# IvanPopov/video-flow-ml

Hardware: AMD Instinct MI355X
Metric: flow-fields/sec @1080p seq5 MOF_sintel (higher is better)
Workload: dtype mixed (per-layer MFMA count, f32 accumulate): {"corr": 1, "update_block.encoder.convf1": 1, "update_block.encoder.convf2": 1, "update_block.gru.convq1.iter": "2a", "update_block.gru.convzr1.iter": 1, "update_block.gru.convzr2.iter": 1, "update_block.mask.0": 1, "update_block.mask.2": 1, "update_bloc

## Files before the change

### include/vfml.h

```cpp
#ifndef VFML_H
#define VFML_H
#include <stddef.h>
#include <stdint.h>

#ifdef __cplusplus
extern "C" {
#endif

#define VFML_ABI_VERSION 25

enum {
  VFML_EPI_NONE = 0,
  VFML_EPI_RELU = 1,
  VFML_EPI_TANH = 2,
  VFML_EPI_SIGMOID = 3,
  VFML_EPI_TANH_RELU = 4,
  VFML_EPI_GRU_ZR = 5,
  VFML_EPI_GRU_Q = 6,
  VFML_EPI_ADD_AUX = 7,
};

enum { VFML_FMT_F32 = 0, VFML_FMT_S16 = 1,
       VFML_FMT_F16 = 2 };

// ... 58 lines not shown
                        const float* res_stats, int n, int hw, int c, float* out, int out_fmt, void* stream);

int vfml_avgpool2x2(const float* x, int n, int h, int w, int c, float* out, void* stream);

int vfml_corr_lookup(const float* const* pyr, const int32_t* hl, const int32_t* wl,
                     const int32_t* ld, int levels, int radius, int nmaps, int q_per_map,
                     const float* coords, int ld_coords, float* out, int ld_out, int out_fmt, int vol_fmt, int vol_tile,
                     void* stream);
#define VFML_VOL_F16_LEVELS(m) (0x100 | (m))

int vfml_corr_lookup_indirect(const float* const* table, const int32_t* hl, const int32_t* wl, const int32_t* ld,
                              int levels, int radius, int nmaps, int q_per_map, const float* coords, int ld_coords,
                              float* out, int ld_out, int out_fmt, int vol_fmt, int vol_tile, void* stream);
int vfml_corr_lookup_indirect_bidir(const float* const* table, const int32_t* hl, const int32_t* wl, const int32_t* ld,
                                    int levels, int radius, int nmaps, int q_per_map, const float* coords, int ld_coords,
                                    int dir_coords, float* out, int ld_out, int dir_out, int dir_tab, int out_fmt, int vol_fmt,
                                    int vol_tile, void* stream);
int vfml_ptr_table_set(void* table, const void* const* ptrs, int n, void* stream);

int vfml_flow_rows7(const float* flow, int n, int h, int w, float* rows, void* stream);

int vfml_conv3x3_c64(const float* in, int ld_in, int n, int h, int w, const void* w_hi, const void* w_lo, int kp, float w_scale,
                     const float* bias, float* out, int ldo, double* stats_part, void* stream);

int vfml_flow_half(const float* flow, int n, int h, int w, const void* w1_hi, int kp1, float w1_scale, const float* b1,
                   const void* w2_hi, int kp2, float w2_scale, const float* b2, float* out, int ld_out, void* stream);

int vfml_tapsum3x3(const float* t, int ld_t, const float* bias, int n, int h, int w, float* out, int parts, int64_t part_stride,
                   void* stream);
int vfml_tapsum3x3_update(const float* t, int ld_t, const float* bias, int n, int h, int w, int parts, int64_t part_stride,
                          float* coords1, float* flow_a, int ld_a, float* flow_b, int ld_b, int fmt_b, void* stream);

int vfml_coords_update(float* coords1, const float* delta, int n, int h, int w,
                       float* flow_a, int ld_a, float* flow_b, int ld_b, int fmt_b, void* stream);
int vfml_coords_init(float* coords1, int n, int h, int w, void* stream);

int vfml_convex_upsample(const float* coords1, int ch, const float* mask, int ld_mask,
                         int h, int w, float* out, void* stream);

int64_t vfml_instnorm_finalize_workspace_bytes(int chunks, int c);
int vfml_instnorm_finalize(const double* part, int n, int chunks, int c, int hw, float eps, float* stats,
                           void* workspace, int64_t workspace_bytes, void* stream);

int vfml_stem7x7s2_chunks(int h, int w);
int vfml_stem7x7s2(const float* frames, int n, int h, int w, const void* w_hi, const void* w_lo, float w_scale,
                   const float* bias, float* out, double* stats_part, void* stream);
// ... 39 lines not shown
```

### video-flow-ml_amd/vfml/csrc/enc_conv.hip

```cpp
#include "conv_split_common.h"

namespace {

constexpr int EC_C = 64;
constexpr int EC_TH = 4, EC_TW = 32;
constexpr int EC_PR = EC_TH + 2, EC_PW = EC_TW + 2;
constexpr int EC_PIX = 272;
constexpr int EC_PATCH = EC_PR * EC_PW * EC_PIX;
constexpr int EC_VLD = EC_C + 4;
constexpr int EC_LDS = EC_PATCH;
constexpr int EC_K = 9 * EC_C;
constexpr int EC_NS = EC_K / 32;
static_assert(EC_TH * EC_TW * EC_VLD * 4 <= EC_PATCH, "the result tile fits where the patch was");

struct EncConvArgs {
  const char* in;
  const _Float16* whi; const _Float16* wlo;
  const float* bias;
  float* out; int ldo;
  double* stats_part;
  int ld_in, n, H, W, tiles_x, tiles_y;
  float w_inv;
};

__global__ __launch_bounds__(256, 2) void enc_conv3x3_c64_kernel(const EncConvArgs a) {
  extern __shared__ __attribute__((aligned(16))) char smem[];
  float* sV = reinterpret_cast<float*>(smem);

  const int t = threadIdx.x, lane = t & 63;
  const int wave = __builtin_amdgcn_readfirstlane(t >> 6);
  const int r4 = lane & 15, u4 = lane >> 4;
  const int tiles_img = a.tiles_x * a.tiles_y;
  const int total = a.n * tiles_img;

  h16x8 bh[EC_NS], bl[EC_NS];
  static_for<EC_NS>([&](auto sc) {
    constexpr int s = decltype(sc)::value;
    bh[s] = *reinterpret_cast<const h16x8*>(a.whi + (16 * wave + r4) * EC_K + s * 32 + u4 * 8);
    bl[s] = *reinterpret_cast<const h16x8*>(a.wlo + (16 * wave + r4) * EC_K + s * 32 + u4 * 8);
  });
  f32x4 bias4 = {0.f, 0.f, 0.f, 0.f};
  if (a.bias) bias4 = *reinterpret_cast<const f32x4*>(a.bias + 16 * wave + 4 * u4);

  for (int tile = blockIdx.x; tile < total; tile += gridDim.x) {
    const int img = tile / tiles_img, tl = tile - img * tiles_img;
    const int ty = tl / a.tiles_x, tx = tl - ty * a.tiles_x;
    const int oy0 = ty * EC_TH, ox0 = tx * EC_TW;

    constexpr int NPC = EC_PR * EC_PW * 16;
    constexpr int NPT = (NPC + 255) / 256;
    const __amdgpu_buffer_rsrc_t rin = __builtin_amdgcn_make_buffer_rsrc(
        const_cast<char*>(a.in) + (int64_t)img * a.H * a.W * a.ld_in * 4, 0, a.H * a.W * a.ld_in * 4, 0x00020000);
    u32x4 pv[NPT];
    static_for<NPT>([&](auto qc) {
      constexpr int q = decltype(qc)::value;
      const int c = min(t + 256 * q, NPC - 1);
      const int p = c >> 4, piece = c & 15;
      const int py = p / EC_PW, px = p - py * EC_PW;
      const int iy = oy0 - 1 + py, ix = ox0 - 1 + px;
      const bool ok = (unsigned)iy < (unsigned)a.H && (unsigned)ix < (unsigned)a.W;
      pv[q] = bload16(rin, ok ? ((iy * a.W + ix) * a.ld_in) * 4 + piece * 16 : (int)0x80000000);
    });
    __syncthreads();
    static_for<NPT>([&](auto qc) {
      constexpr int q = decltype(qc)::value;
      const int c = t + 256 * q;
      if (c < NPC) *reinterpret_cast<u32x4*>(smem + (c >> 4) * EC_PIX + (c & 15) * 16) = pv[q];
    });
    __syncthreads();

    f32x4 acc[8];
#pragma unroll
    for (int m = 0; m < 8; ++m) acc[m] = f32x4{0.f, 0.f, 0.f, 0.f};
    const char* al = smem + r4 * EC_PIX + u4 * 32;
    static_for<2>([&](auto hc) {
      constexpr int mh = decltype(hc)::value;
      static_for<EC_NS>([&](auto sc) {
        constexpr int s = decltype(sc)::value;
        constexpr int cb = s / 9, ky = (s % 9) / 3, kx = s % 3;
#pragma unroll
        for (int mm = 0; mm < 4; ++mm) {
          const int m = 4 * mh + mm;
          const char* p = al + (((m >> 1) + ky) * EC_PW + 16 * (m & 1) + kx) * EC_PIX + cb * 128;
          const h16x8 ah = *reinterpret_cast<const h16x8*>(p);
          const h16x8 alo = *reinterpret_cast<const h16x8*>(p + 16);
          acc[m] = __builtin_amdgcn_mfma_f32_16x16x32_f16(bh[s], ah, acc[m], 0, 0, 0);
          acc[m] = __builtin_amdgcn_mfma_f32_16x16x32_f16(bl[s], ah, acc[m], 0, 0, 0);
          acc[m] = __builtin_amdgcn_mfma_f32_16x16x32_f16(bh[s], alo, acc[m], 0, 0, 0);
        }
        if constexpr (s % 3 == 2) __builtin_amdgcn_sched_barrier(0);
// ... 17 lines not shown
      __syncthreads();
      const int row = t >> 6, ch = t & 63;
      const int oy = oy0 + row;
      if (oy < a.H) {
        double s1 = 0.0, s2 = 0.0;
        for (int x = 0; x < EC_TW; ++x) {
          float f = sV[(row * EC_TW + x) * EC_VLD + ch], g;
          asm("v_mov_b32 %0, %1" : "=v"(g) : "v"(f));
          const double v = (double)g;
          s1 += v;
          s2 += v * v;
        }
        const int64_t chunk = (((int64_t)img * a.H + oy) * a.W + ox0) >> 5;
        double* o = a.stats_part + (chunk * EC_C + ch) * 2;
        o[0] = s1;
        o[1] = s2;
      }
    }
  }
}

}

extern "C" int vfml_conv3x3_c64(const float* in, int ld_in, int n, int h, int w, const void* w_hi, const void* w_lo, int kp,
                                float w_scale, const float* bias, float* out, int ldo, double* stats_part, void* stream) {
  VFML_REQUIRE(in && w_hi && w_lo && out && n > 0 && h > 0 && w > 0, "vfml_conv3x3_c64: bad argument");
  VFML_REQUIRE(w % EC_TW == 0, "vfml_conv3x3_c64: the image width must be a multiple of %d (got %d)", EC_TW, w);
  VFML_REQUIRE(kp == EC_K && w_scale > 0.f, "vfml_conv3x3_c64: weight planes [64][%d] (VFML_KORDER_CBLOCK), got row pitch %d", EC_K, kp);
  VFML_REQUIRE((reinterpret_cast<uintptr_t>(in) & 31u) == 0 && ld_in >= EC_C && ld_in % 8 == 0 && vfml_aligned16(w_hi) &&
                   vfml_aligned16(w_lo) && vfml_aligned16(bias) && vfml_aligned16(out) && ldo >= EC_C && ldo % 4 == 0 &&
                   (reinterpret_cast<uintptr_t>(stats_part) & 7u) == 0,
               "vfml_conv3x3_c64: a 32-byte aligned split-row input (ld_in %% 8 == 0), 16-byte aligned weights / bias / output "
               "(ldo %% 4 == 0)");
  EncConvArgs a;
  a.in = reinterpret_cast<const char*>(in); a.ld_in = ld_in;
  a.whi = reinterpret_cast<const _Float16*>(w_hi); a.wlo = reinterpret_cast<const _Float16*>(w_lo);
  a.bias = bias; a.out = out; a.ldo = ldo; a.stats_part = stats_part;
  a.n = n; a.H = h; a.W = w; a.tiles_x = w / EC_TW; a.tiles_y = (h + EC_TH - 1) / EC_TH;
  a.w_inv = 1.0f / w_scale;
  const int64_t total = (int64_t)n * a.tiles_x * a.tiles_y;
  VFML_REQUIRE(total < (1ll << 31) && (int64_t)h * w * ld_in * 4 < (1ll << 31), "vfml_conv3x3_c64: an image of the input must stay below 2 GiB");
  const int grid = (int)(total < 512 ? total : 512);
  hipLaunchKernelGGL(enc_conv3x3_c64_kernel, dim3(grid), dim3(256), EC_LDS, reinterpret_cast<hipStream_t>(stream), a);
  return vfml_check_launch("vfml_conv3x3_c64");
}
```

### video-flow-ml_amd/vfml/csrc/norm_pool.hip

```cpp
#include <stdlib.h>
#include "vfml_common.h"

namespace {

__global__ void frames_u8_kernel(const uint8_t* __restrict__ src, int64_t npx, float scale, float shift,
                                 f32x4* __restrict__ dst) {
  for (int64_t p = (int64_t)blockIdx.x * blockDim.x + threadIdx.x; p < npx; p += (int64_t)gridDim.x * blockDim.x) {
    const uint8_t* s = src + p * 3;
    f32x4 v;
    v[0] = scale * ((float)s[0] / 255.0f) + shift;
    v[1] = scale * ((float)s[1] / 255.0f) + shift;
    v[2] = scale * ((float)s[2] / 255.0f) + shift;
    v[3] = 0.f;
    dst[p] = v;
  }
}

__global__ void frames_f32_kernel(const float* __restrict__ src, int n, int64_t hw, float scale, float shift,
                                  f32x4* __restrict__ dst) {
  const int64_t npx = (int64_t)n * hw;
  for (int64_t p = (int64_t)blockIdx.x * blockDim.x + threadIdx.x; p < npx; p += (int64_t)gridDim.x * blockDim.x) {
    const int64_t f = p / hw, q = p - f * hw;
    const float* s = src + f * 3 * hw + q;
    f32x4 v;
// ... 34 lines not shown
  extern __shared__ __attribute__((aligned(16))) char smem_raw[];
  double* sh = reinterpret_cast<double*>(smem_raw);
  if (pl < lanes) {
#pragma unroll
    for (int e = 0; e < 4; ++e) {
      sh[((int64_t)pl * c + g * 4 + e) * 2 + 0] = s[e];
      sh[((int64_t)pl * c + g * 4 + e) * 2 + 1] = q[e];
    }
  }
  __syncthreads();
  for (int ch = t; ch < c; ch += STAT_THREADS) {
    double ss = 0, qq = 0;
    for (int l = 0; l < lanes; ++l) {
      ss += vfml_lds_f64(&sh[((int64_t)l * c + ch) * 2 + 0]);
      qq += vfml_lds_f64(&sh[((int64_t)l * c + ch) * 2 + 1]);
    }
    double* o = part + (((int64_t)n * gridDim.x + chunk) * c + ch) * 2;
    o[0] = ss;
    o[1] = qq;
  }
}

constexpr int FINAL_THREADS = 256;
__global__ __launch_bounds__(FINAL_THREADS) void instnorm_final_kernel(const double* __restrict__ part, int n, int chunks,
                                                                      int c, int hw, float eps, float* __restrict__ stats) {
  __shared__ double sh[FINAL_THREADS][2];
  const int i = blockIdx.x;
  const int nn = i / c, ch = i - nn * c;
  const int t = threadIdx.x;
  const double* base = part + ((int64_t)nn * chunks * c + ch) * 2;
  double s = 0, q = 0;
  int k = t;
  for (; k + 3 * FINAL_THREADS < chunks; k += 4 * FINAL_THREADS) {
    const double* p0 = base + (int64_t)k * c * 2;
    const double* p1 = p0 + (int64_t)FINAL_THREADS * c * 2;
    const double* p2 = p1 + (int64_t)FINAL_THREADS * c * 2;
    const double* p3 = p2 + (int64_t)FINAL_THREADS * c * 2;
    const double a0 = p0[0], b0 = p0[1], a1 = p1[0], b1 = p1[1], a2 = p2[0], b2 = p2[1], a3 = p3[0], b3 = p3[1];
    s += a0; q += b0; s += a1; q += b1; s += a2; q += b2; s += a3; q += b3;
  }
  for (; k < chunks; k += FINAL_THREADS) {
    const double* p = base + (int64_t)k * c * 2;
    s += p[0];
    q += p[1];
  }
  sh[t][0] = s;
  sh[t][1] = q;
  __syncthreads();
  if (t == 0) {
    double ss = 0, qq = 0;
    for (int l = 0; l < FINAL_THREADS; ++l) {
      ss += vfml_lds_f64(&sh[l][0]);
      qq += vfml_lds_f64(&sh[l][1]);
    }
    const double mean = ss / hw;
    double var = qq / hw - mean * mean;
    if (var < 0) var = 0;
    stats[2 * i + 0] = (float)mean;
    stats[2 * i + 1] = (float)(1.0 / sqrt(var + (double)eps));
  }
}

constexpr int FOLD_SLICES = 64;
__global__ __launch_bounds__(256) void instnorm_fold_kernel(const double* __restrict__ part, int chunks, int c,
                                                            double* __restrict__ out) {
  __shared__ double sh[32][8][2];
  const int cgs = c / 8;
  const int sl = blockIdx.x % FOLD_SLICES, cg = (blockIdx.x / FOLD_SLICES) % cgs, nn = blockIdx.x / (FOLD_SLICES * cgs);
  const int ch = threadIdx.x & 7, lane = threadIdx.x >> 3;
  const int per = (chunks + FOLD_SLICES - 1) / FOLD_SLICES;
  const int k0 = sl * per, k1 = k0 + per < chunks ? k0 + per : chunks;
  const double* base = part + ((int64_t)nn * chunks * c + cg * 8 + ch) * 2;
  double s0 = 0, q0 = 0;
  for (int k = k0 + lane; k < k1; k += 32) {
    const double* p = base + (int64_t)k * c * 2;
    s0 += p[0];
    q0 += p[1];
  }
  sh[lane][ch][0] = s0;
  sh[lane][ch][1] = q0;
  __syncthreads();
  if (lane == 0) {
// ... 105 lines not shown
  return vfml_check_launch("vfml_frames_to_nhwc4");
}

extern "C" int64_t vfml_instnorm_workspace_bytes(int n, int hw, int c) {
  return (int64_t)n * stat_chunks(hw) * c * 2 * sizeof(double);
}

extern "C" int vfml_instnorm_stats(const float* x, int n, int hw, int c, float eps, float* stats, void* workspace,
                                   void* stream) {
  VFML_REQUIRE(x && stats && workspace, "vfml_instnorm_stats: null pointer");
  VFML_REQUIRE(n > 0 && hw > 0 && c > 0 && c % 4 == 0 && c <= 1024, "vfml_instnorm_stats: bad n/hw/c (c%%4==0, c<=1024)");
  VFML_REQUIRE(vfml_aligned16(x), "vfml_instnorm_stats: x must be 16-byte aligned");
  hipStream_t s = reinterpret_cast<hipStream_t>(stream);
  const int chunks = stat_chunks(hw);
  const int px = (hw + chunks - 1) / chunks;
  const int lanes = STAT_THREADS / (c / 4);
  VFML_REQUIRE(lanes >= 1, "vfml_instnorm_stats: too many channels");
  const size_t lds = (size_t)lanes * c * 2 * sizeof(double);
  VFML_REQUIRE(lds <= 64 * 1024, "vfml_instnorm_stats: LDS budget");
  hipLaunchKernelGGL(instnorm_partial_kernel, dim3(chunks, n), dim3(STAT_THREADS), lds, s, x, hw, c, px,
                     (double*)workspace);
  int rc = vfml_check_launch("vfml_instnorm_stats(partial)");
  if (rc) return rc;
  hipLaunchKernelGGL(instnorm_final_kernel, dim3(n * c), dim3(FINAL_THREADS), 0, s, (const double*)workspace, n, chunks, c, hw,
                     eps, stats);
  return vfml_check_launch("vfml_instnorm_stats(final)");
}

static bool finalize_folds(int chunks, int c) { return chunks >= 1024 && c % 8 == 0; }

extern "C" int64_t vfml_instnorm_finalize_workspace_bytes(int chunks, int c) {
  return finalize_folds(chunks, c) ? (int64_t)FOLD_SLICES * c * 16 : 0;
}

extern "C" int vfml_instnorm_finalize(const double* part, int n, int chunks, int c, int hw, float eps, float* stats,
                                      void* workspace, int64_t workspace_bytes, void* stream) {
  VFML_REQUIRE(part && stats && n > 0 && chunks > 0 && c > 0 && hw > 0, "vfml_instnorm_finalize: bad argument");
  hipStream_t st = reinterpret_cast<hipStream_t>(stream);
  if (finalize_folds(chunks, c)) {
    const int64_t per_frame = (int64_t)FOLD_SLICES * c * 16;
    VFML_REQUIRE(workspace && workspace_bytes >= per_frame && (reinterpret_cast<uintptr_t>(workspace) & 15u) == 0,
                 "vfml_instnorm_finalize: %d partials x %d channels fold through a workspace of >= %lld bytes (16-byte aligned); got %lld",
                 chunks, c, (long long)per_frame, (long long)(workspace ? workspace_bytes : 0));
    const int nmax = (int)(workspace_bytes / per_frame);
    for (int n0 = 0; n0 < n; n0 += nmax) {
      const int nb = n - n0 < nmax ? n - n0 : nmax;
      hipLaunchKernelGGL(instnorm_fold_kernel, dim3(nb * (c / 8) * FOLD_SLICES), dim3(256), 0, st,
                         part + (int64_t)n0 * chunks * c * 2, chunks, c, (double*)workspace);
      hipLaunchKernelGGL(instnorm_final_kernel, dim3(nb * c), dim3(FINAL_THREADS), 0, st, (const double*)workspace, nb,
                         FOLD_SLICES, c, hw, eps, stats + (int64_t)n0 * c * 2);
    }
    return vfml_check_launch("vfml_instnorm_finalize");
  }
  hipLaunchKernelGGL(instnorm_final_kernel, dim3(n * c), dim3(FINAL_THREADS), 0, st, part, n, chunks,
                     c, hw, eps, stats);
  return vfml_check_launch("vfml_instnorm_finalize");
}

extern "C" int vfml_instnorm_apply(const float* x, const float* stats, const float* res, const float* res_stats, int n,
                                   int hw, int c, float* out, int out_fmt, void* stream) {
  VFML_REQUIRE(x && stats && out, "vfml_instnorm_apply: null pointer");
  VFML_REQUIRE(n > 0 && hw > 0 && c > 0 && c % 4 == 0, "vfml_instnorm_apply: bad n/hw/c");
  VFML_REQUIRE(out_fmt == VFML_FMT_F32 || (out_fmt == VFML_FMT_S16 && c % 8 == 0 && (reinterpret_cast<uintptr_t>(out) & 31u) == 0 &&
                                            (!res || res_stats || (reinterpret_cast<uintptr_t>(res) & 31u) == 0)),
               "vfml_instnorm_apply: split-row output needs c %% 8 == 0 and 32-byte aligned out (and res)");
  VFML_REQUIRE(!(res_stats && !res), "vfml_instnorm_apply: res_stats without res");
  VFML_REQUIRE(vfml_aligned16(x) && vfml_aligned16(out) && vfml_aligned16(res), "vfml_instnorm_apply: alignment");
  hipStream_t s = reinterpret_cast<hipStream_t>(stream);
  const int64_t total4 = (int64_t)n * hw * (c / 4);
  const dim3 g(grid_for(total4, 256)), b(256);
  const bool s16 = out_fmt == VFML_FMT_S16;
#define VFML_APPLY(MODE, S16, R, RS)                                                                                      \
  hipLaunchKernelGGL((instnorm_apply_kernel<MODE, S16>), g, b, 0, s, (const f32x4*)x, stats, (const f32x4*)(R), RS, hw, c, \
                     total4, (f32x4*)out)
  if (!res) {
    if (s16) VFML_APPLY(0, true, nullptr, nullptr); else VFML_APPLY(0, false, nullptr, nullptr);
  } else if (!res_stats) {
// ... 19 lines not shown
```

### video-flow-ml_amd/vfml/hip.py

```python
import ctypes
import os
import subprocess
from ctypes import POINTER, c_char_p, c_double, c_float, c_int, c_int32, c_int64, c_void_p

import torch

_HERE = os.path.dirname(os.path.abspath(__file__))
LIB_PATH = os.environ.get("VFML_LIB") or os.path.join(_HERE, "libvfml_hip.so")
CSRC = os.path.join(_HERE, "csrc")
SOURCES = ["api.hip", "conv_gemm.hip", "conv_gemm_split.hip", "conv_gemm_tapx.hip", "stem.hip", "flow_half.hip", "enc_conv.hip", "norm_pool.hip", "flow_ops.hip", "effects.hip", "correct.hip", "render.hip"]

STATS_ROWS_F32, STATS_ROWS_S16 = 128, 32
EPI_NONE, EPI_RELU, EPI_TANH, EPI_SIGMOID, EPI_TANH_RELU, EPI_GRU_ZR, EPI_GRU_Q, EPI_ADD_AUX = range(8)
FMT_F32, FMT_S16, FMT_F16 = 0, 1, 2


def vol_f16_levels(mask):
    return 0x100 | mask


def _vol_mask(vol_fmt, levels):
    return (15 if vol_fmt == FMT_F16 else (vol_fmt & 15 if vol_fmt & 0x100 else 0)) & ((1 << levels) - 1)

KORDER_TAP, KORDER_CBLOCK, KORDER_CBLOCK64 = 0, 1, 2
# ... 86 lines not shown
    L.vfml_softmax_rows_f16.argtypes = [c_void_p, c_int64, c_int, c_int64, c_void_p, c_int64, c_float, c_void_p]
    L.vfml_transpose_to_s16.argtypes = [c_void_p, c_int, c_int, c_int, c_float, c_void_p, c_int64, c_void_p]
    L.vfml_add_to_s16.argtypes = [c_void_p, c_int64, c_void_p, c_int64, c_void_p, c_int64, c_int64, c_int, c_float, c_void_p]
    L.vfml_instnorm_finalize.argtypes = [c_void_p, c_int, c_int, c_int, c_int, c_float, c_void_p, c_void_p, c_int64, c_void_p]
    L.vfml_instnorm_finalize_workspace_bytes.restype = c_int64
    L.vfml_instnorm_finalize_workspace_bytes.argtypes = [c_int, c_int]
    L.vfml_stem7x7s2_chunks.argtypes = [c_int, c_int]
    L.vfml_stem7x7s2.argtypes = [c_void_p, c_int, c_int, c_int, c_void_p, c_void_p, c_float, c_void_p, c_void_p, c_void_p, c_void_p]
    L.vfml_instnorm_apply.argtypes = [c_void_p, c_void_p, c_void_p, c_void_p, c_int, c_int, c_int, c_void_p, c_int, c_void_p]
    L.vfml_avgpool2x2.argtypes = [c_void_p, c_int, c_int, c_int, c_int, c_void_p, c_void_p]
    L.vfml_corr_lookup.argtypes = [POINTER(c_void_p), POINTER(c_int32), POINTER(c_int32), POINTER(c_int32),
                                   c_int, c_int, c_int, c_int, c_void_p, c_int, c_void_p, c_int, c_int, c_int, c_int, c_void_p]
    L.vfml_corr_lookup_indirect.argtypes = [c_void_p, POINTER(c_int32), POINTER(c_int32), POINTER(c_int32),
                                            c_int, c_int, c_int, c_int, c_void_p, c_int, c_void_p, c_int, c_int, c_int, c_int,
                                            c_void_p]
    L.vfml_corr_lookup_indirect_bidir.argtypes = [c_void_p, POINTER(c_int32), POINTER(c_int32), POINTER(c_int32),
                                                  c_int, c_int, c_int, c_int, c_void_p, c_int, c_int, c_void_p, c_int, c_int,
                                                  c_int, c_int, c_int, c_int, c_void_p]
    L.vfml_ptr_table_set.argtypes = [c_void_p, POINTER(c_void_p), c_int, c_void_p]
    L.vfml_tapsum3x3_update.argtypes = [c_void_p, c_int, c_void_p, c_int, c_int, c_int, c_int, ctypes.c_int64, c_void_p, c_void_p,
                                        c_int, c_void_p, c_int, c_int, c_void_p]
    L.vfml_conv3x3_c64.argtypes = [c_void_p, c_int, c_int, c_int, c_int, c_void_p, c_void_p, c_int, c_float, c_void_p, c_void_p,
                                   c_int, c_void_p, c_void_p]
    L.vfml_flow_half.argtypes = [c_void_p, c_int, c_int, c_int, c_void_p, c_int, c_float, c_void_p, c_void_p, c_int, c_float,
                                 c_void_p, c_void_p, c_int, c_void_p]
    L.vfml_coords_init.argtypes = [c_void_p, c_int, c_int, c_int, c_void_p]
    L.vfml_flow_rows7.argtypes = [c_void_p, c_int, c_int, c_int, c_void_p, c_void_p]
    L.vfml_tapsum3x3.argtypes = [c_void_p, c_int, c_void_p, c_int, c_int, c_int, c_void_p, c_int, ctypes.c_int64, c_void_p]
    L.vfml_coords_update.argtypes = [c_void_p, c_void_p, c_int, c_int, c_int, c_void_p, c_int, c_void_p, c_int,
                                     c_int, c_void_p]
    L.vfml_flow_lod.argtypes = [c_void_p, c_int, c_int, c_void_p, c_void_p]
    L.vfml_flow_encode.argtypes = [c_void_p, c_int, c_int, c_int, c_float, c_float, c_float, c_float, c_float, c_void_p,
                                   c_void_p]
    L.vfml_taa_blend.argtypes = [c_void_p, c_int, c_void_p, c_void_p, c_int, c_void_p, c_int, c_int, c_int, c_int, c_double,
                                 c_double, c_void_p]
    L.vfml_flow_quality_map.argtypes = [c_void_p, c_void_p, c_void_p, c_int, c_int, c_int, c_int, c_float, c_void_p, c_void_p]
    L.vfml_flow_correct_workspace_bytes.argtypes = [c_int, c_int]
    L.vfml_flow_correct_workspace_bytes.restype = ctypes.c_size_t
    L.vfml_flow_correct.argtypes = [c_void_p, c_void_p, c_void_p, c_void_p, c_int, c_int, c_int, c_int, c_void_p,
                                    c_double, c_double, c_double, c_double, c_double, c_void_p, c_void_p, c_void_p,
                                    ctypes.c_int64, c_void_p, ctypes.c_size_t, c_void_p]
    L.vfml_flow_colorize.argtypes = [c_void_p, c_int, c_int, c_int, c_void_p, c_void_p, c_void_p]
    L.vfml_compose_frame.argtypes = [POINTER(c_void_p), POINTER(c_int32), c_int, c_int, c_int, c_int, c_int64, c_void_p,
                                     c_void_p]
    L.vfml_convex_upsample.argtypes = [c_void_p, c_int, c_void_p, c_int, c_int, c_int, c_void_p, c_void_p]
    for name in EXPORTS:
        getattr(L, name)
    if L.vfml_abi_version() != 25:
        raise RuntimeError("libvfml_hip.so ABI version mismatch")
    _lib = L
    return L


EXPORTS = [
    "vfml_conv2d", "vfml_conv2d_split", "vfml_split_f16", "vfml_to_s16", "vfml_softmax_rows_s16", "vfml_softmax_rows_f16", "vfml_transpose_to_s16", "vfml_add_to_s16",
    "vfml_transpose_split_f16", "vfml_frames_to_nhwc4", "vfml_instnorm_workspace_bytes", "vfml_instnorm_stats",
    "vfml_instnorm_apply", "vfml_instnorm_finalize", "vfml_instnorm_finalize_workspace_bytes", "vfml_avgpool2x2", "vfml_corr_lookup", "vfml_corr_lookup_indirect", "vfml_corr_lookup_indirect_bidir",
    "vfml_ptr_table_set", "vfml_coords_update", "vfml_coords_init", "vfml_tapsum3x3", "vfml_tapsum3x3_update", "vfml_flow_rows7", "vfml_flow_half", "vfml_conv3x3_c64",
    "vfml_convex_upsample", "vfml_stem7x7s2", "vfml_stem7x7s2_chunks", "vfml_flow_lod", "vfml_flow_encode", "vfml_taa_blend", "vfml_flow_quality_map", "vfml_flow_correct_workspace_bytes", "vfml_flow_correct",
    "vfml_flow_colorize", "vfml_compose_frame",
    "vfml_last_error", "vfml_abi_version",
]


def _check(rc, what):
    if rc != 0:
        raise RuntimeError(f"{what} failed (rc={rc}): {lib().vfml_last_error().decode()}")


def _stream():
    return c_void_p(torch.cuda.current_stream().cuda_stream)


def _ptr(t, offset=0):
    if t is None:
        return None
    return c_void_p(t.data_ptr() + 4 * offset)


def _dev(t, dtype=torch.float32):
    if not (t.is_cuda and t.dtype == dtype and t.is_contiguous()):
# ... 376 lines not shown


def coords_init(coords1, n, h, w):
    _check(lib().vfml_coords_init(_ptr(_dev(coords1)), n, h, w, _stream()), "vfml_coords_init")


def flow_rows7(flow, n, h, w, rows):
    _check(lib().vfml_flow_rows7(_ptr(_dev(flow)), n, h, w, _ptr(_dev(rows)), _stream()), "vfml_flow_rows7")


def tapsum3x3(t, ld_t, bias, n, h, w, out, parts=1, part_stride=0):
    _check(lib().vfml_tapsum3x3(_ptr(_dev(t)), ld_t, _ptr(bias) if bias is not None else None, n, h, w, _ptr(_dev(out)),
                                parts, part_stride, _stream()), "vfml_tapsum3x3")


def conv3x3_c64(src, ld_in, n, h, w, weight, bias, out, ldo, stats_part=None, src_off=0):
    _check(lib().vfml_conv3x3_c64(_ptr(_dev(src), src_off), ld_in, n, h, w, c_void_p(weight.hi.data_ptr()),
                                  c_void_p(weight.lo.data_ptr()), weight.kp, weight.scale,
                                  _ptr(_dev(bias)) if bias is not None else None, _ptr(_dev(out)), ldo,
                                  c_void_p(stats_part.data_ptr()) if stats_part is not None else None, _stream()),
           "vfml_conv3x3_c64")


def flow_half(flow, n, h, w, w1, b1, w2, b2, out, ld_out, out_off=0):
    _check(lib().vfml_flow_half(_ptr(_dev(flow)), n, h, w, c_void_p(w1.hi.data_ptr()), w1.kp, w1.scale, _ptr(_dev(b1)),
                                c_void_p(w2.hi.data_ptr()), w2.kp, w2.scale, _ptr(_dev(b2)), _ptr(_dev(out), out_off), ld_out,
                                _stream()), "vfml_flow_half")


def tapsum3x3_update(t, ld_t, bias, n, h, w, coords1, parts=1, part_stride=0, flow_a=None, ld_a=0, flow_a_off=0, flow_b=None,
                     ld_b=0, flow_b_off=0, fmt_b=FMT_F32):
    _check(lib().vfml_tapsum3x3_update(_ptr(_dev(t)), ld_t, _ptr(bias) if bias is not None else None, n, h, w, parts, part_stride,
                                       _ptr(_dev(coords1)), _ptr(flow_a, flow_a_off), ld_a, _ptr(flow_b, flow_b_off), ld_b,
                                       fmt_b, _stream()), "vfml_tapsum3x3_update")


def coords_update(coords1, delta, n, h, w, flow_a=None, ld_a=0, flow_a_off=0, flow_b=None, ld_b=0, flow_b_off=0,
                  fmt_b=FMT_F32):
    _check(lib().vfml_coords_update(_ptr(_dev(coords1)), _ptr(delta), n, h, w,
                                    _ptr(flow_a, flow_a_off), ld_a, _ptr(flow_b, flow_b_off), ld_b, fmt_b, _stream()),
           "vfml_coords_update")


def flow_lods(flow, num_lods=5):
    lods = [_dev(flow.contiguous())]
    for _ in range(1, num_lods):
# ... 139 lines not shown
```

### video-flow-ml_amd/vfml/network.py

```python
import os

import torch
import torch.nn as nn

from . import hip
from .weights import conv_spec, corr_channel_subset, pack_conv_weight


def cor_pad(cor, split):
    return (cor + 15) // 16 * 16 if split else (cor + 3) // 4 * 4


def take_frames(src, idx):
    idx = list(idx)
    if all(b == a + 1 for a, b in zip(idx, idx[1:])):
        return src[idx[0]:idx[0] + len(idx)]
    return torch.stack([src[i] for i in idx])


class _Holder(nn.Module):

    def child(self, name):
        if name not in self._modules:
            self.add_module(name, _Holder())
# ... 267 lines not shown
        st.replay()

    def _encoder(self, prefix, x, n, H, W, P, dev, out, ldo, out_off, epilogue, split, out_fmt=hip.FMT_F32):
        h2, w2 = H // 2, W // 2
        big = n * h2 * w2 * 64
        raw = self._buf("enc_raw", big, dev)
        raw2 = self._buf("enc_raw2", big, dev)
        act = [self._buf("enc_act0", big, dev), self._buf("enc_act1", big, dev), self._buf("enc_act2", big, dev)]
        st = self._buf("enc_stats", 3 * n * 128 * 2, dev)
        nws = hip.instnorm_workspace_bytes(n, h2 * w2, 128)
        ws = self._buf("enc_statws", (nws + 7) // 8, dev, torch.float64)

        def stats_of(t, hw, c, slot):
            s = st[slot * n * 128 * 2:]
            hip.instnorm_stats(t, n, hw, c, s, ws)
            return s

        split_prec = self._split()
        AF = hip.FMT_S16 if split_prec else hip.FMT_F32
        part_len = n * ((h2 * w2 + 31) // 32) * 64 * 2
        parts = self._buf("enc_part", 3 * part_len, dev, torch.float64) if split_prec else None
        fold_ws = self._buf("enc_foldws", min(n, 8) * 64 * 128 * 2, dev, torch.float64) if split_prec else None

        def conv_stats(src, c, hh_, ww_, name, planes, dst, slot, k, stride=1, pad=0, src_fmt=hip.FMT_F32):
            wgt, b = P[name]
            nm = self._nm(name) if split_prec else 3
            ho_, wo_ = (hh_ + 2 * pad - k) // stride + 1, (ww_ + 2 * pad - k) // stride + 1
            hw = ho_ * wo_
            rows = hip.STATS_ROWS_S16 if src_fmt == hip.FMT_S16 else hip.STATS_ROWS_F32
            if not (split_prec and (n == 1 or hw % rows == 0)):
                hip.conv2d(src, c, c, n, hh_, ww_, wgt, b, planes, k, k, dst, planes, stride=stride, pad_h=pad, pad_w=pad,
                           mfma=nm, in_fmt=src_fmt)
                return stats_of(dst, hw, planes, slot)
            chunks = (hw + rows - 1) // rows
            part = parts[slot * part_len:]
            if (c == 64 and planes == 64 and k == 3 and stride == 1 and pad == 1 and nm == 3 and src_fmt == hip.FMT_S16
                    and ww_ % 32 == 0 and getattr(wgt, "order", None) == hip.KORDER_CBLOCK and wgt.kp == 576 and wgt.lo is not None):
                hip.conv3x3_c64(src, c, n, hh_, ww_, wgt, b, dst, planes, stats_part=part)
            else:
                hip.conv2d(src, c, c, n, hh_, ww_, wgt, b, planes, k, k, dst, planes, stride=stride, pad_h=pad, pad_w=pad,
                           stats_part=part, mfma=nm, in_fmt=src_fmt)
            s = st[slot * n * 128 * 2:]
            hip.instnorm_finalize(part, n, chunks, planes, hw, s, workspace=fold_ws)
            return s

        stem = P.get(f"{prefix}.conv1.stem")
        if stem is not None and split_prec and self._nm(f"{prefix}.conv1") == 3:
            chunks = hip.stem_chunks(H, W)
            part = parts[0:]
            hip.stem7x7s2(x, n, H, W, stem[0], stem[1], raw, stats_part=part)
            s0 = st[0:]
            hip.instnorm_finalize(part, n, chunks, 64, h2 * w2, s0, workspace=fold_ws)
        else:
            s0 = conv_stats(x, 4, H, W, f"{prefix}.conv1", 64, raw, 0, 7, stride=2, pad=3)
        cur = act[0]
        hip.instnorm_apply(raw, s0, n, h2 * w2, 64, cur, out_fmt=AF)
        ch, hh, ww, ci = 64, h2, w2, 0
        for li, (planes, stride) in enumerate([(64, 1), (96, 2), (128, 2)], start=1):
            for bi in range(2):
                stv = stride if bi == 0 else 1
                ho, wo = (hh, ww) if stv == 1 else ((hh - 1) // 2 + 1, (ww - 1) // 2 + 1)
                name = f"{prefix}.layer{li}.{bi}"
                y = act[(ci + 1) % 3]
                nxt = act[(ci + 2) % 3]
                s1 = conv_stats(cur, ch, hh, ww, f"{name}.conv1", planes, raw, 0, 3, stride=stv, pad=1, src_fmt=AF)
                hip.instnorm_apply(raw, s1, n, ho * wo, planes, y, out_fmt=AF)
                s2 = conv_stats(y, planes, ho, wo, f"{name}.conv2", planes, raw, 1, 3, pad=1, src_fmt=AF)
                if stv != 1:
                    s3 = conv_stats(cur, ch, hh, ww, f"{name}.downsample.0", planes, raw2, 2, 1, stride=stv, src_fmt=AF)
                    hip.instnorm_apply(raw, s2, n, ho * wo, planes, nxt, res=raw2, res_stats=s3, out_fmt=AF)
                else:
                    hip.instnorm_apply(raw, s2, n, ho * wo, planes, nxt, res=cur, out_fmt=AF)
                cur, ci = nxt, (ci + 2) % 3
                ch, hh, ww = planes, ho, wo
        wgt, b = P[f"{prefix}.conv2"]
        hip.conv2d(cur, 128, 128, n, hh, ww, wgt, b, 256, 1, 1, out, ldo, out_off=out_off, epilogue=epilogue,
                   split=split, out_fmt=out_fmt, in_fmt=AF, mfma=self._nm(f"{prefix}.conv2") if split_prec else 3)
        return hh, ww

    @torch.no_grad()
    def forward(self, images, data=None, return_lowres=True):
        if not isinstance(images, torch.Tensor) or not images.is_cuda:
            raise RuntimeError("MOFNetHIP runs on an MI355X (HIP) device only; got "
                               f"{getattr(images, 'device', type(images))}. There is no CPU fallback in the shipped engine.")
        if images.dim() != 5 or images.shape[2] != 3:
            raise ValueError(f"images must be [B,N,3,H,W], got {tuple(images.shape)}")
        if images.shape[0] != 1:
            raise ValueError(f"Batch size must be 1, got {images.shape[0]}")
        src = images[0]
        if src.dtype != torch.float32:
            src = src.float()
        return self._run(src.contiguous(), src.shape[0], src.shape[2], src.shape[3], return_lowres)

    @torch.no_grad()
    def forward_u8(self, frames, return_lowres=True, frame_keys=None, tri_batch=False, pick_only=False):
# ... 475 lines not shown
```

Before: 44.50.

## Fuse instance-norm apply into the 64-channel 3x3 conv input load; parallelize stats finalize

Adds a NORM variant of the encoder 3x3 c64 conv that reads the raw f32 conv1 output plus its instance-norm statistics. It normalizes, applies ReLU and splits to f16 hi/lo while staging the input patch in LDS. This skips the separate instnorm_apply pass and the write and reread of the normalized activation for layer1 conv2. The stats finalize kernel is also restructured so each block reduces 8 channels at once instead of one channel per block. The trade-off is reading f32 input with twice the bytes of the split format, extra ALU work in the load stage, and more LDS per block.

```diff
diff --git a/include/vfml.h b/include/vfml.h
--- a/include/vfml.h
+++ b/include/vfml.h
@@ -104,6 +104,9 @@
 
 int vfml_conv3x3_c64(const float* in, int ld_in, int n, int h, int w, const void* w_hi, const void* w_lo, int kp, float w_scale,
                      const float* bias, float* out, int ldo, double* stats_part, void* stream);
+int vfml_conv3x3_c64_norm(const float* raw, const float* raw_stats, int ld_in, int n, int h, int w, const void* w_hi,
+                          const void* w_lo, int kp, float w_scale, const float* bias, float* out, int ldo, double* stats_part,
+                          void* stream);
 
 int vfml_flow_half(const float* flow, int n, int h, int w, const void* w1_hi, int kp1, float w1_scale, const float* b1,
                    const void* w2_hi, int kp2, float w2_scale, const float* b2, float* out, int ld_out, void* stream);
diff --git a/video-flow-ml_amd/vfml/csrc/enc_conv.hip b/video-flow-ml_amd/vfml/csrc/enc_conv.hip
--- a/video-flow-ml_amd/vfml/csrc/enc_conv.hip
+++ b/video-flow-ml_amd/vfml/csrc/enc_conv.hip
@@ -9,12 +9,14 @@
 constexpr int EC_PATCH = EC_PR * EC_PW * EC_PIX;
 constexpr int EC_VLD = EC_C + 4;
 constexpr int EC_LDS = EC_PATCH;
+constexpr int EC_LDS_NORM = EC_PATCH + EC_C * 8;
 constexpr int EC_K = 9 * EC_C;
 constexpr int EC_NS = EC_K / 32;
 static_assert(EC_TH * EC_TW * EC_VLD * 4 <= EC_PATCH, "the result tile fits where the patch was");
 
 struct EncConvArgs {
   const char* in;
+  const float* nstats;
   const _Float16* whi; const _Float16* wlo;
   const float* bias;
   float* out; int ldo;
@@ -23,6 +25,7 @@
   float w_inv;
 };
 
+template <bool NORM>
 __global__ __launch_bounds__(256, 2) void enc_conv3x3_c64_kernel(const EncConvArgs a) {
   extern __shared__ __attribute__((aligned(16))) char smem[];
   float* sV = reinterpret_cast<float*>(smem);
@@ -42,6 +45,7 @@
   f32x4 bias4 = {0.f, 0.f, 0.f, 0.f};
   if (a.bias) bias4 = *reinterpret_cast<const f32x4*>(a.bias + 16 * wave + 4 * u4);
 
+  int stats_img = -1;
   for (int tile = blockIdx.x; tile < total; tile += gridDim.x) {
     const int img = tile / tiles_img, tl = tile - img * tiles_img;
     const int ty = tl / a.tiles_x, tx = tl - ty * a.tiles_x;
@@ -52,20 +56,55 @@
     const __amdgpu_buffer_rsrc_t rin = __builtin_amdgcn_make_buffer_rsrc(
         const_cast<char*>(a.in) + (int64_t)img * a.H * a.W * a.ld_in * 4, 0, a.H * a.W * a.ld_in * 4, 0x00020000);
     u32x4 pv[NPT];
+    int ts = t;
+    if constexpr (NORM) asm volatile("" : "+v"(ts));
+    unsigned okm = 0;
+    if constexpr (NORM) {
+      if (img != stats_img) {
+        if (t < EC_C / 2)
+          *reinterpret_cast<f32x4*>(smem + EC_PATCH + 16 * t) = *reinterpret_cast<const f32x4*>(a.nstats + (int64_t)img * EC_C * 2 + 4 * t);
+        stats_img = img;
+      }
+    }
     static_for<NPT>([&](auto qc) {
       constexpr int q = decltype(qc)::value;
-      const int c = min(t + 256 * q, NPC - 1);
+      const int c = min(ts + 256 * q, NPC - 1);
       const int p = c >> 4, piece = c & 15;
       const int py = p / EC_PW, px = p - py * EC_PW;
       const int iy = oy0 - 1 + py, ix = ox0 - 1 + px;
       const bool ok = (unsigned)iy < (unsigned)a.H && (unsigned)ix < (unsigned)a.W;
       pv[q] = bload16(rin, ok ? ((iy * a.W + ix) * a.ld_in) * 4 + piece * 16 : (int)0x80000000);
+      if constexpr (NORM) okm |= ok ? 1u << q : 0u;
     });
     __syncthreads();
+    f32x4 mr0, mr1;
+    if constexpr (NORM) {
+      mr0 = *reinterpret_cast<const f32x4*>(smem + EC_PATCH + (t & 15) * 32);
+      mr1 = *reinterpret_cast<const f32x4*>(smem + EC_PATCH + (t & 15) * 32 + 16);
+    }
     static_for<NPT>([&](auto qc) {
       constexpr int q = decltype(qc)::value;
       const int c = t + 256 * q;
-      if (c < NPC) *reinterpret_cast<u32x4*>(smem + (c >> 4) * EC_PIX + (c & 15) * 16) = pv[q];
+      if constexpr (!NORM) {
+        if (c < NPC) *reinterpret_cast<u32x4*>(smem + (c >> 4) * EC_PIX + (c & 15) * 16) = pv[q];
+      } else {
+        const f32x4 v = __builtin_bit_cast(f32x4, pv[q]);
+        const float o0 = fmaxf((v[0] - mr0[0]) * mr0[1], 0.f), o1 = fmaxf((v[1] - mr0[2]) * mr0[3], 0.f);
+        const float o2 = fmaxf((v[2] - mr1[0]) * mr1[1], 0.f), o3 = fmaxf((v[3] - mr1[2]) * mr1[3], 0.f);
+        vfml_h16x2 h0, h1, l0, l1;
+        vfml_split2(o0, o1, h0, l0);
+        vfml_split2(o2, o3, h1, l1);
+        const bool ok = (okm >> q) & 1u;
+        uint2 hv, lv;
+        hv.x = ok ? __builtin_bit_cast(unsigned, h0) : 0u; hv.y = ok ? __builtin_bit_cast(unsigned, h1) : 0u;
+        lv.x = ok ? __builtin_bit_cast(unsigned, l0) : 0u; lv.y = ok ? __builtin_bit_cast(unsigned, l1) : 0u;
+        char* u = smem + (c >> 4) * EC_PIX + ((c & 15) >> 1) * 32 + (c & 1) * 8;
+        if (c < NPC) {
+          *reinterpret_cast<uint2*>(u) = hv;
+          *reinterpret_cast<uint2*>(u + 16) = lv;
+        }
+        __builtin_amdgcn_sched_barrier(0);
+      }
     });
     __syncthreads();
 
@@ -129,25 +168,45 @@
 
 }
 
-extern "C" int vfml_conv3x3_c64(const float* in, int ld_in, int n, int h, int w, const void* w_hi, const void* w_lo, int kp,
-                                float w_scale, const float* bias, float* out, int ldo, double* stats_part, void* stream) {
-  VFML_REQUIRE(in && w_hi && w_lo && out && n > 0 && h > 0 && w > 0, "vfml_conv3x3_c64: bad argument");
-  VFML_REQUIRE(w % EC_TW == 0, "vfml_conv3x3_c64: the image width must be a multiple of %d (got %d)", EC_TW, w);
-  VFML_REQUIRE(kp == EC_K && w_scale > 0.f, "vfml_conv3x3_c64: weight planes [64][%d] (VFML_KORDER_CBLOCK), got row pitch %d", EC_K, kp);
-  VFML_REQUIRE((reinterpret_cast<uintptr_t>(in) & 31u) == 0 && ld_in >= EC_C && ld_in % 8 == 0 && vfml_aligned16(w_hi) &&
+static int enc_conv_launch(const char* who, const float* in, const float* nstats, int ld_in, int n, int h, int w, const void* w_hi,
+                           const void* w_lo, int kp, float w_scale, const float* bias, float* out, int ldo, double* stats_part,
+                           void* stream) {
+  const bool norm = nstats != nullptr;
+  VFML_REQUIRE(in && w_hi && w_lo && out && n > 0 && h > 0 && w > 0, "%s: bad argument", who);
+  VFML_REQUIRE(w % EC_TW == 0, "%s: the image width must be a multiple of %d (got %d)", who, EC_TW, w);
+  VFML_REQUIRE(kp == EC_K && w_scale > 0.f, "%s: weight planes [64][%d] (VFML_KORDER_CBLOCK), got row pitch %d", who, EC_K, kp);
+  VFML_REQUIRE((reinterpret_cast<uintptr_t>(in) & (norm ? 15u : 31u)) == 0 && ld_in >= EC_C && ld_in % (norm ? 4 : 8) == 0 &&
+                   vfml_aligned16(nstats) && vfml_aligned16(w_hi) &&
                    vfml_aligned16(w_lo) && vfml_aligned16(bias) && vfml_aligned16(out) && ldo >= EC_C && ldo % 4 == 0 &&
                    (reinterpret_cast<uintptr_t>(stats_part) & 7u) == 0,
-               "vfml_conv3x3_c64: a 32-byte aligned split-row input (ld_in %% 8 == 0), 16-byte aligned weights / bias / output "
-               "(ldo %% 4 == 0)");
+               "%s: a 32-byte aligned split-row input (ld_in %% 8 == 0) or 16-byte aligned f32 rows and statistics (ld_in %% 4 == 0), "
+               "16-byte aligned weights / bias / output (ldo %% 4 == 0)", who);
   EncConvArgs a;
-  a.in = reinterpret_cast<const char*>(in); a.ld_in = ld_in;
+  a.in = reinterpret_cast<const char*>(in); a.nstats = nstats; a.ld_in = ld_in;
   a.whi = reinterpret_cast<const _Float16*>(w_hi); a.wlo = reinterpret_cast<const _Float16*>(w_lo);
   a.bias = bias; a.out = out; a.ldo = ldo; a.stats_part = stats_part;
   a.n = n; a.H = h; a.W = w; a.tiles_x = w / EC_TW; a.tiles_y = (h + EC_TH - 1) / EC_TH;
   a.w_inv = 1.0f / w_scale;
   const int64_t total = (int64_t)n * a.tiles_x * a.tiles_y;
-  VFML_REQUIRE(total < (1ll << 31) && (int64_t)h * w * ld_in * 4 < (1ll << 31), "vfml_conv3x3_c64: an image of the input must stay below 2 GiB");
+  VFML_REQUIRE(total < (1ll << 31) && (int64_t)h * w * ld_in * 4 < (1ll << 31), "%s: an image of the input must stay below 2 GiB", who);
   const int grid = (int)(total < 512 ? total : 512);
-  hipLaunchKernelGGL(enc_conv3x3_c64_kernel, dim3(grid), dim3(256), EC_LDS, reinterpret_cast<hipStream_t>(stream), a);
-  return vfml_check_launch("vfml_conv3x3_c64");
-}
+  if (norm)
+    hipLaunchKernelGGL(enc_conv3x3_c64_kernel<true>, dim3(grid), dim3(256), EC_LDS_NORM, reinterpret_cast<hipStream_t>(stream), a);
+  else
+    hipLaunchKernelGGL(enc_conv3x3_c64_kernel<false>, dim3(grid), dim3(256), EC_LDS, reinterpret_cast<hipStream_t>(stream), a);
+  return vfml_check_launch(who);
+}
+
+extern "C" int vfml_conv3x3_c64(const float* in, int ld_in, int n, int h, int w, const void* w_hi, const void* w_lo, int kp,
+                                float w_scale, const float* bias, float* out, int ldo, double* stats_part, void* stream) {
+  return enc_conv_launch("vfml_conv3x3_c64", in, nullptr, ld_in, n, h, w, w_hi, w_lo, kp, w_scale, bias, out, ldo, stats_part, stream);
+}
+
+extern "C" int vfml_conv3x3_c64_norm(const float* raw, const float* raw_stats, int ld_in, int n, int h, int w, const void* w_hi,
+                                     const void* w_lo, int kp, float w_scale, const float* bias, float* out, int ldo,
+                                     double* stats_part, void* stream) {
+  VFML_REQUIRE(raw_stats, "vfml_conv3x3_c64_norm: null statistics");
+  VFML_REQUIRE(raw != out, "vfml_conv3x3_c64_norm: in place (a tile reads its neighbours' input rows)");
+  return enc_conv_launch("vfml_conv3x3_c64_norm", raw, raw_stats, ld_in, n, h, w, w_hi, w_lo, kp, w_scale, bias, out, ldo,
+                         stats_part, stream);
+}
diff --git a/video-flow-ml_amd/vfml/csrc/norm_pool.hip b/video-flow-ml_amd/vfml/csrc/norm_pool.hip
--- a/video-flow-ml_amd/vfml/csrc/norm_pool.hip
+++ b/video-flow-ml_amd/vfml/csrc/norm_pool.hip
@@ -80,42 +80,64 @@
 }
 
 constexpr int FINAL_THREADS = 256;
-__global__ __launch_bounds__(FINAL_THREADS) void instnorm_final_kernel(const double* __restrict__ part, int n, int chunks,
-                                                                      int c, int hw, float eps, float* __restrict__ stats) {
-  __shared__ double sh[FINAL_THREADS][2];
-  const int i = blockIdx.x;
-  const int nn = i / c, ch = i - nn * c;
-  const int t = threadIdx.x;
-  const double* base = part + ((int64_t)nn * chunks * c + ch) * 2;
-  double s = 0, q = 0;
-  int k = t;
-  for (; k + 3 * FINAL_THREADS < chunks; k += 4 * FINAL_THREADS) {
-    const double* p0 = base + (int64_t)k * c * 2;
-    const double* p1 = p0 + (int64_t)FINAL_THREADS * c * 2;
-    const double* p2 = p1 + (int64_t)FINAL_THREADS * c * 2;
-    const double* p3 = p2 + (int64_t)FINAL_THREADS * c * 2;
-    const double a0 = p0[0], b0 = p0[1], a1 = p1[0], b1 = p1[1], a2 = p2[0], b2 = p2[1], a3 = p3[0], b3 = p3[1];
-    s += a0; q += b0; s += a1; q += b1; s += a2; q += b2; s += a3; q += b3;
-  }
-  for (; k < chunks; k += FINAL_THREADS) {
-    const double* p = base + (int64_t)k * c * 2;
-    s += p[0];
-    q += p[1];
-  }
-  sh[t][0] = s;
-  sh[t][1] = q;
+constexpr int FIN_CH = 8, FIN_LANES = FINAL_THREADS / FIN_CH, FIN_PER = FINAL_THREADS / FIN_LANES;
+__global__ __launch_bounds__(FINAL_THREADS) void instnorm_final_kernel(const double* __restrict__ part, int chunks, int c, int hw,
+                                                                      float eps, float* __restrict__ stats) {
+  __shared__ double sh[FINAL_THREADS][FIN_CH][2];
+  const int cgs = (c + FIN_CH - 1) / FIN_CH;
+  const int nn = blockIdx.x / cgs, cg = blockIdx.x - nn * cgs;
+  const int t = threadIdx.x, ch = t & (FIN_CH - 1), lane = t >> 3;
+  const bool live = cg * FIN_CH + ch < c;
+  const double* base = part + ((int64_t)nn * chunks * c + cg * FIN_CH + ch) * 2;
+  double s[FIN_PER], q[FIN_PER];
+#pragma unroll
+  for (int j = 0; j < FIN_PER; ++j) s[j] = q[j] = 0;
+  if (live) {
+    for (int k0 = 0; k0 < chunks; k0 += FINAL_THREADS) {
+      double a[FIN_PER], b[FIN_PER];
+#pragma unroll
+      for (int j = 0; j < FIN_PER; ++j) {
+        const int k = k0 + lane + FIN_LANES * j;
+        const double* p = base + (int64_t)(k < chunks ? k : 0) * c * 2;
+        a[j] = p[0];
+        b[j] = p[1];
+      }
+#pragma unroll
+      for (int j = 0; j < FIN_PER; ++j)
+        if (k0 + lane + FIN_LANES * j < chunks) {
+          s[j] += a[j];
+          q[j] += b[j];
+        }
+    }
+  }
+#pragma unroll
+  for (int j = 0; j < FIN_PER; ++j) {
+    sh[lane + FIN_LANES * j][ch][0] = s[j];
+    sh[lane + FIN_LANES * j][ch][1] = q[j];
+  }
   __syncthreads();
-  if (t == 0) {
+  if (t < FIN_CH && live) {
+    const int nt = chunks < FINAL_THREADS ? (chunks + 7) & ~7 : FINAL_THREADS;
     double ss = 0, qq = 0;
-    for (int l = 0; l < FINAL_THREADS; ++l) {
-      ss += vfml_lds_f64(&sh[l][0]);
-      qq += vfml_lds_f64(&sh[l][1]);
+    for (int l0 = 0; l0 < nt; l0 += 8) {
+      double a[8], b[8];
+#pragma unroll
+      for (int i = 0; i < 8; ++i) {
+        a[i] = vfml_lds_f64(&sh[l0 + i][ch][0]);
+        b[i] = vfml_lds_f64(&sh[l0 + i][ch][1]);
+      }
+#pragma unroll
+      for (int i = 0; i < 8; ++i) {
+        ss += a[i];
+        qq += b[i];
+      }
     }
     const double mean = ss / hw;
     double var = qq / hw - mean * mean;
     if (var < 0) var = 0;
-    stats[2 * i + 0] = (float)mean;
-    stats[2 * i + 1] = (float)(1.0 / sqrt(var + (double)eps));
+    float* st = stats + ((int64_t)nn * c + cg * FIN_CH + ch) * 2;
+    st[0] = (float)mean;
+    st[1] = (float)(1.0 / sqrt(var + (double)eps));
   }
 }
 
@@ -267,8 +289,8 @@
                      (double*)workspace);
   int rc = vfml_check_launch("vfml_instnorm_stats(partial)");
   if (rc) return rc;
-  hipLaunchKernelGGL(instnorm_final_kernel, dim3(n * c), dim3(FINAL_THREADS), 0, s, (const double*)workspace, n, chunks, c, hw,
-                     eps, stats);
+  hipLaunchKernelGGL(instnorm_final_kernel, dim3(n * ((c + FIN_CH - 1) / FIN_CH)), dim3(FINAL_THREADS), 0, s,
+                     (const double*)workspace, chunks, c, hw, eps, stats);
   return vfml_check_launch("vfml_instnorm_stats(final)");
 }
 
@@ -292,12 +314,12 @@
       const int nb = n - n0 < nmax ? n - n0 : nmax;
       hipLaunchKernelGGL(instnorm_fold_kernel, dim3(nb * (c / 8) * FOLD_SLICES), dim3(256), 0, st,
                          part + (int64_t)n0 * chunks * c * 2, chunks, c, (double*)workspace);
-      hipLaunchKernelGGL(instnorm_final_kernel, dim3(nb * c), dim3(FINAL_THREADS), 0, st, (const double*)workspace, nb,
+      hipLaunchKernelGGL(instnorm_final_kernel, dim3(nb * (c / FIN_CH)), dim3(FINAL_THREADS), 0, st, (const double*)workspace,
                          FOLD_SLICES, c, hw, eps, stats + (int64_t)n0 * c * 2);
     }
     return vfml_check_launch("vfml_instnorm_finalize");
   }
-  hipLaunchKernelGGL(instnorm_final_kernel, dim3(n * c), dim3(FINAL_THREADS), 0, st, part, n, chunks,
+  hipLaunchKernelGGL(instnorm_final_kernel, dim3(n * ((c + FIN_CH - 1) / FIN_CH)), dim3(FINAL_THREADS), 0, st, part, chunks,
                      c, hw, eps, stats);
   return vfml_check_launch("vfml_instnorm_finalize");
 }
diff --git a/video-flow-ml_amd/vfml/hip.py b/video-flow-ml_amd/vfml/hip.py
--- a/video-flow-ml_amd/vfml/hip.py
+++ b/video-flow-ml_amd/vfml/hip.py
@@ -132,6 +132,8 @@
                                         c_int, c_void_p, c_int, c_int, c_void_p]
     L.vfml_conv3x3_c64.argtypes = [c_void_p, c_int, c_int, c_int, c_int, c_void_p, c_void_p, c_int, c_float, c_void_p, c_void_p,
                                    c_int, c_void_p, c_void_p]
+    L.vfml_conv3x3_c64_norm.argtypes = [c_void_p, c_void_p, c_int, c_int, c_int, c_int, c_void_p, c_void_p, c_int, c_float, c_void_p,
+                                        c_void_p, c_int, c_void_p, c_void_p]
     L.vfml_flow_half.argtypes = [c_void_p, c_int, c_int, c_int, c_void_p, c_int, c_float, c_void_p, c_void_p, c_int, c_float,
                                  c_void_p, c_void_p, c_int, c_void_p]
     L.vfml_coords_init.argtypes = [c_void_p, c_int, c_int, c_int, c_void_p]
@@ -166,7 +168,7 @@
     "vfml_conv2d", "vfml_conv2d_split", "vfml_split_f16", "vfml_to_s16", "vfml_softmax_rows_s16", "vfml_softmax_rows_f16", "vfml_transpose_to_s16", "vfml_add_to_s16",
     "vfml_transpose_split_f16", "vfml_frames_to_nhwc4", "vfml_instnorm_workspace_bytes", "vfml_instnorm_stats",
     "vfml_instnorm_apply", "vfml_instnorm_finalize", "vfml_instnorm_finalize_workspace_bytes", "vfml_avgpool2x2", "vfml_corr_lookup", "vfml_corr_lookup_indirect", "vfml_corr_lookup_indirect_bidir",
-    "vfml_ptr_table_set", "vfml_coords_update", "vfml_coords_init", "vfml_tapsum3x3", "vfml_tapsum3x3_update", "vfml_flow_rows7", "vfml_flow_half", "vfml_conv3x3_c64",
+    "vfml_ptr_table_set", "vfml_coords_update", "vfml_coords_init", "vfml_tapsum3x3", "vfml_tapsum3x3_update", "vfml_flow_rows7", "vfml_flow_half", "vfml_conv3x3_c64", "vfml_conv3x3_c64_norm",
     "vfml_convex_upsample", "vfml_stem7x7s2", "vfml_stem7x7s2_chunks", "vfml_flow_lod", "vfml_flow_encode", "vfml_taa_blend", "vfml_flow_quality_map", "vfml_flow_correct_workspace_bytes", "vfml_flow_correct",
     "vfml_flow_colorize", "vfml_compose_frame",
     "vfml_last_error", "vfml_abi_version",
@@ -589,6 +591,14 @@
            "vfml_conv3x3_c64")
 
 
+def conv3x3_c64_norm(raw, raw_stats, ld_in, n, h, w, weight, bias, out, ldo, stats_part=None):
+    _check(lib().vfml_conv3x3_c64_norm(_ptr(_dev(raw)), _ptr(_dev(raw_stats)), ld_in, n, h, w, c_void_p(weight.hi.data_ptr()),
+                                       c_void_p(weight.lo.data_ptr()), weight.kp, weight.scale,
+                                       _ptr(_dev(bias)) if bias is not None else None, _ptr(_dev(out)), ldo,
+                                       c_void_p(stats_part.data_ptr()) if stats_part is not None else None, _stream()),
+           "vfml_conv3x3_c64_norm")
+
+
 def flow_half(flow, n, h, w, w1, b1, w2, b2, out, ld_out, out_off=0):
     _check(lib().vfml_flow_half(_ptr(_dev(flow)), n, h, w, c_void_p(w1.hi.data_ptr()), w1.kp, w1.scale, _ptr(_dev(b1)),
                                 c_void_p(w2.hi.data_ptr()), w2.kp, w2.scale, _ptr(_dev(b2)), _ptr(_dev(out), out_off), ld_out,
diff --git a/video-flow-ml_amd/vfml/network.py b/video-flow-ml_amd/vfml/network.py
--- a/video-flow-ml_amd/vfml/network.py
+++ b/video-flow-ml_amd/vfml/network.py
@@ -313,7 +313,11 @@
         parts = self._buf("enc_part", 3 * part_len, dev, torch.float64) if split_prec else None
         fold_ws = self._buf("enc_foldws", min(n, 8) * 64 * 128 * 2, dev, torch.float64) if split_prec else None
 
-        def conv_stats(src, c, hh_, ww_, name, planes, dst, slot, k, stride=1, pad=0, src_fmt=hip.FMT_F32):
+        def c64_kernel(c, planes, k, stride, pad, nm, ww_, wgt):
+            return (c == 64 and planes == 64 and k == 3 and stride == 1 and pad == 1 and nm == 3 and ww_ % 32 == 0
+                    and getattr(wgt, "order", None) == hip.KORDER_CBLOCK and wgt.kp == 576 and wgt.lo is not None)
+
+        def conv_stats(src, c, hh_, ww_, name, planes, dst, slot, k, stride=1, pad=0, src_fmt=hip.FMT_F32, src_stats=None):
             wgt, b = P[name]
             nm = self._nm(name) if split_prec else 3
             ho_, wo_ = (hh_ + 2 * pad - k) // stride + 1, (ww_ + 2 * pad - k) // stride + 1
@@ -325,8 +329,9 @@
                 return stats_of(dst, hw, planes, slot)
             chunks = (hw + rows - 1) // rows
             part = parts[slot * part_len:]
-            if (c == 64 and planes == 64 and k == 3 and stride == 1 and pad == 1 and nm == 3 and src_fmt == hip.FMT_S16
-                    and ww_ % 32 == 0 and getattr(wgt, "order", None) == hip.KORDER_CBLOCK and wgt.kp == 576 and wgt.lo is not None):
+            if src_stats is not None:
+                hip.conv3x3_c64_norm(src, src_stats, c, n, hh_, ww_, wgt, b, dst, planes, stats_part=part)
+            elif src_fmt == hip.FMT_S16 and c64_kernel(c, planes, k, stride, pad, nm, ww_, wgt):
                 hip.conv3x3_c64(src, c, n, hh_, ww_, wgt, b, dst, planes, stats_part=part)
             else:
                 hip.conv2d(src, c, c, n, hh_, ww_, wgt, b, planes, k, k, dst, planes, stride=stride, pad_h=pad, pad_w=pad,
@@ -355,13 +360,20 @@
                 y = act[(ci + 1) % 3]
                 nxt = act[(ci + 2) % 3]
                 s1 = conv_stats(cur, ch, hh, ww, f"{name}.conv1", planes, raw, 0, 3, stride=stv, pad=1, src_fmt=AF)
-                hip.instnorm_apply(raw, s1, n, ho * wo, planes, y, out_fmt=AF)
-                s2 = conv_stats(y, planes, ho, wo, f"{name}.conv2", planes, raw, 1, 3, pad=1, src_fmt=AF)
+                w2_ = P[f"{name}.conv2"][0]
+                if (split_prec and stv == 1 and (n == 1 or (ho * wo) % hip.STATS_ROWS_S16 == 0)
+                        and c64_kernel(planes, planes, 3, 1, 1, self._nm(f"{name}.conv2"), wo, w2_)):
+                    r2 = raw2
+                    s2 = conv_stats(raw, planes, ho, wo, f"{name}.conv2", planes, r2, 1, 3, pad=1, src_fmt=AF, src_stats=s1)
+                else:
+                    r2 = raw
+                    hip.instnorm_apply(raw, s1, n, ho * wo, planes, y, out_fmt=AF)
+                    s2 = conv_stats(y, planes, ho, wo, f"{name}.conv2", planes, r2, 1, 3, pad=1, src_fmt=AF)
                 if stv != 1:
                     s3 = conv_stats(cur, ch, hh, ww, f"{name}.downsample.0", planes, raw2, 2, 1, stride=stv, src_fmt=AF)
-                    hip.instnorm_apply(raw, s2, n, ho * wo, planes, nxt, res=raw2, res_stats=s3, out_fmt=AF)
+                    hip.instnorm_apply(r2, s2, n, ho * wo, planes, nxt, res=raw2, res_stats=s3, out_fmt=AF)
                 else:
-                    hip.instnorm_apply(raw, s2, n, ho * wo, planes, nxt, res=cur, out_fmt=AF)
+                    hip.instnorm_apply(r2, s2, n, ho * wo, planes, nxt, res=cur, out_fmt=AF)
                 cur, ci = nxt, (ci + 2) % 3
                 ch, hh, ww = planes, ho, wo
         wgt, b = P[f"{prefix}.conv2"]
```

Result: no change. 44.87, median of 6 (+0.8%).
